# beyzoskaya/HiC-GNN

Measured on AMD Instinct MI355X. Metric: training steps/sec (GATNetSelectiveResidualsUpdated, fwd+loss+bwd+Adam), higher is better.
Workload: dtype fp32; 1 GPU; synth-20000; n_nodes=20000, nnz_with_self_loops=4019956, d=512, heads=2, loss=mse, parallelism=single, gemm=fp32 MFMA

## Files before the change

### hic-gnn_amd/csrc/gat_bwd.hip

```cpp
#include <algorithm>
#include <cstdlib>

#include "gat_agg.hpp"
#include "gat_launch.hpp"

namespace hicgat {

__global__ __launch_bounds__(256) void agg_bwd_dst_h2c256_kernel(
    const int *__restrict__ rowptr, const int *__restrict__ col, int row_begin, int row_end,
    const float *__restrict__ h, const float *__restrict__ a_src, const float *__restrict__ a_dst,
    const float *__restrict__ dout, float ns, float *__restrict__ row_stats) {
  const int i = row_begin + xcd_remap(blockIdx.x, gridDim.x) * 4 + wave_in_block();
  if (i < row_end) agg_bwd_dst_row<2, 256>(i, rowptr, col, h, a_src, a_dst, dout, ns, row_stats);
}

template <int H, int C>
__global__ __launch_bounds__(256) void agg_bwd_dst_generic_kernel(
    const int *__restrict__ rowptr, const int *__restrict__ col, int row_begin, int row_end,
    const float *__restrict__ h, const float *__restrict__ a_src, const float *__restrict__ a_dst,
    const float *__restrict__ dout, float ns, float *__restrict__ row_stats) {
  const int i = row_begin + xcd_remap(blockIdx.x, gridDim.x) * 4 + wave_in_block();
  if (i >= row_end) return;
  agg_bwd_dst_row<H, C>(i, rowptr, col, h, a_src, a_dst, dout, ns, row_stats);
}

template <bool SPLIT = false, bool REMAP = true, class... MK>
__global__ __launch_bounds__(256) void agg_bwd_src_h2c256_kernel(
    const int *__restrict__ rowptr, const int *__restrict__ col, int row_begin, int row_end,
    const float *__restrict__ h, const float *__restrict__ a_src, const float *__restrict__ a_dst,
    const float *__restrict__ row_stats, int64_t ldr, const float *__restrict__ dout, int64_t ldq,
    const float *__restrict__ att_s, const float *__restrict__ att_d, float ns,
    float *__restrict__ dh, float *__restrict__ da_src, MK... mk) {
  const int r = row_begin + (REMAP ? xcd_remap(blockIdx.x, gridDim.x) : (int)blockIdx.x) * 4 + wave_in_block();
  if (r < row_end)
    agg_bwd_src_row<2, 256, SPLIT, sizeof...(MK) != 0>(r, rowptr, col, h, a_src, a_dst, row_stats, ldr, dout, ldq,
                                                       att_s, att_d, ns, dh, da_src, mk...);
}

template <int H, int C, bool REMAP, class... MK>
__global__ __launch_bounds__(256) void agg_bwd_src_generic_kernel(
    const int *__restrict__ rowptr, const int *__restrict__ col, int row_begin, int row_end,
    const float *__restrict__ h, const float *__restrict__ a_src, const float *__restrict__ a_dst,
    const float *__restrict__ row_stats, int64_t ldr, const float *__restrict__ dout, int64_t ldq,
    const float *__restrict__ att_s, const float *__restrict__ att_d, float ns,
    float *__restrict__ dh, float *__restrict__ da_src, MK... mk) {
  const int r = row_begin + (REMAP ? xcd_remap(blockIdx.x, gridDim.x) : (int)blockIdx.x) * 4 + wave_in_block();
  if (r >= row_end) return;
  agg_bwd_src_row<H, C, false, sizeof...(MK) != 0>(r, rowptr, col, h, a_src, a_dst, row_stats, ldr, dout, ldq, att_s,
                                                   att_d, ns, dh, da_src, mk...);
}

template <int ACT>
__global__ __launch_bounds__(256) void agg_bwd_rows_kernel(int row_begin, int row_end,
                                                           const float *__restrict__ g,
                                                           const float *__restrict__ y,
                                                           const float *__restrict__ bias,
                                                           const float *__restrict__ out2,
                                                           float *__restrict__ dout, int64_t ldq,
                                                           float *__restrict__ row_stats) {
  const int i = row_begin + blockIdx.x * 4 + wave_in_block();
  if (i < row_end) agg_bwd_rows_row<2, 256, ACT>(i, g, y, bias, out2, dout, ldq, row_stats);
}

template <int H, int C, int ACT>
__global__ __launch_bounds__(256) void agg_bwd_rows_generic_kernel(int row_begin, int row_end,
                                                                   const float *__restrict__ g,
                                                                   const float *__restrict__ y,
                                                                   const float *__restrict__ bias,
                                                                   const float *__restrict__ out2,
                                                                   float *__restrict__ dout, int64_t ldq,
                                                                   float *__restrict__ row_stats) {
  const int i = row_begin + blockIdx.x * 4 + wave_in_block();
  if (i >= row_end) return;
  agg_bwd_rows_row<H, C, ACT>(i, g, y, bias, out2, dout, ldq, row_stats);
}

constexpr int kParamBlocks = 512;

template <int PARTS>
__global__ __launch_bounds__(256) void param_grad_stage1(const float *__restrict__ h,
                                                         const float *__restrict__ dout,
                                                         const float *__restrict__ da_src,
                                                         const float *__restrict__ row_stats, int N,
                                                         int H, int C, int rows_per_block,
                                                         float *__restrict__ part) {
  constexpr bool kS = PARTS & 1, kT = PARTS & 2, kB = PARTS & 4;
  constexpr int P = (int)kS + (int)kT + (int)kB;
  const int D = H * C, Q = D / 4;
  const int r0 = blockIdx.x * rows_per_block, r1 = min(N, r0 + rows_per_block);
  const float4 *h4 = reinterpret_cast<const float4 *>(h);
  const float4 *g4 = reinterpret_cast<const float4 *>(dout);
  float4 *p4 = reinterpret_cast<float4 *>(part + (size_t)blockIdx.x * P * D);
  for (int q = threadIdx.x; q < Q; q += blockDim.x) {
    const int hd = (4 * q) / C;
    float4 s = make_float4(0.f, 0.f, 0.f, 0.f), t = s, b = s;
#pragma unroll 4
    for (int n = r0; n < r1; ++n) {
      if (kS || kT) {
        const float4 hv = h4[(size_t)n * Q + q];
        if (kS) s = f4_fma(da_src[(size_t)n * H + hd], hv, s);
        if (kT) t = f4_fma(row_stats[(size_t)n * 4 * H + 3 * H + hd], hv, t);
      }
      if (kB) {
        const float4 gv = g4[(size_t)n * Q + q];
        b.x += gv.x; b.y += gv.y; b.z += gv.z; b.w += gv.w;
      }
    }
    int o = 0;
    if (kS) p4[(o++) * Q + q] = s;
    if (kT) p4[(o++) * Q + q] = t;
    if (kB) p4[o * Q + q] = b;
  }
}

constexpr int kPG2Groups = 16, kPG2Cols = 16;
struct PGOut {
  float *o[3];
};
__global__ __launch_bounds__(256) void param_grad_stage2(const float *__restrict__ part, int nblk, int P, int D,
                                                         PGOut out, int accumulate) {
  __shared__ float red[kPG2Groups][kPG2Cols];
  const int cl = threadIdx.x % kPG2Cols, grp = threadIdx.x / kPG2Cols;
  const int c = blockIdx.x * kPG2Cols + cl;
  float s = 0.f;
  if (c < P * D) {
    constexpr int kMax = (kParamBlocks + kPG2Groups - 1) / kPG2Groups;
    float v[kMax];
#pragma unroll
    for (int i = 0; i < kMax; ++i) {
      const int b = grp + i * kPG2Groups;
      v[i] = b < nblk ? part[(size_t)b * P * D + c] : 0.f;
    }
#pragma unroll
    for (int i = 0; i < kMax; ++i) s += v[i];
  }
  red[grp][cl] = s;
  __syncthreads();
  if (grp == 0 && c < P * D) {
    float t = red[0][cl];
#pragma unroll
    for (int g = 1; g < kPG2Groups; ++g) t += red[g][cl];
    float *o = out.o[c / D] + c % D;
    *o = t + (accumulate ? *o : 0.f);
  }
}

constexpr size_t kSrcOccLds = 32768;

int agg_bwd_src_split_launch(const int *rowptr_s, const int *col_s, int row_begin, int row_end, const float *h,
                             const float *a_src, const float *a_dst, const float *row_stats, int64_t ldr,
                             const float *dout, int64_t ldq4, float ns, float *dh, float *da_src, hipStream_t s) {
  hipLaunchKernelGGL((agg_bwd_src_h2c256_kernel<true>), dim3((row_end - row_begin + 3) / 4), dim3(256), 0, s,
                     rowptr_s, col_s, row_begin, row_end, h, a_src, a_dst, row_stats, ldr, dout, ldq4, nullptr, nullptr,
                     ns, dh, da_src);
  HICGAT_CHECK_LAUNCH();
  return HICGAT_OK;
}

template <class... MK>
int agg_bwd_src_launch(const int *rowptr, const int *col, int H, int C, int row_begin, int row_end, const float *h,
                       const float *a_src, const float *a_dst, const float *row_stats, int64_t ldr, const float *dout,
                       int64_t ldq4, const float *att_s, const float *att_d, float ns, float *dh, float *da_src,
                       bool remap, hipStream_t s, MK... mk) {
  const dim3 grid((row_end - row_begin + 3) / 4), block(256);
  return for_gat_shape(H, C, [&](auto shape) {
    return with_flags(
        [&](auto rm) {
          using S = decltype(shape);
          constexpr bool REMAP = rm.value;
          if constexpr (S::h2c256)
            hipLaunchKernelGGL((agg_bwd_src_h2c256_kernel<false, REMAP, MK...>), grid, block,
                               REMAP && !sizeof...(MK) ? kSrcOccLds : 0, s, rowptr, col, row_begin, row_end, h, a_src,
                               a_dst, row_stats, ldr, dout, ldq4, att_s, att_d, ns, dh, da_src, mk...);
          else
            hipLaunchKernelGGL((agg_bwd_src_generic_kernel<S::H, S::C, REMAP, MK...>), grid, block, 0, s, rowptr, col,
                               row_begin, row_end, h, a_src, a_dst, row_stats, ldr, dout, ldq4, att_s, att_d, ns, dh,
                               da_src, mk...);
          HICGAT_CHECK_LAUNCH();
          return HICGAT_OK;
        },
        remap);
  });
}

static int agg_bwd_src_checked(const int32_t *rowptr, const int32_t *col, int N, int H, int C, int row_begin,
                               int row_end, const float *h, const float *a_src, const float *a_dst,
                               const float *row_stats, int64_t ld_stats, const float *dout, int64_t ld_dout,
                               const float *att_src, const float *att_dst, float neg_slope, float *dh, float *da_src,
                               int flags, const AttnMaskArgs *mk, hipStream_t s) {
  if (flags & ~HICGAT_SRC_ROUND_ROBIN) return HICGAT_EINVAL;
  const bool remap = !(flags & HICGAT_SRC_ROUND_ROBIN);
  if (N < 0 || row_begin < 0 || row_end > N || row_begin > row_end) return HICGAT_EINVAL;
  if (!gat_shape_supported(H, C)) return HICGAT_EUNSUPPORTED;
  if (ld_stats < 4 * H || ld_stats % 4 || ld_dout < H * C || ld_dout % 4) return HICGAT_EINVAL;
  if (row_end == row_begin) return HICGAT_OK;
  if (!rowptr || !col || !h || !a_src || !a_dst || !row_stats || !dout || !att_src || !att_dst ||
      !dh || !da_src)
    return HICGAT_EINVAL;
  if (mk)
    return agg_bwd_src_launch(rowptr, col, H, C, row_begin, row_end, h, a_src, a_dst, row_stats, ld_stats, dout,
                              ld_dout / 4, att_src, att_dst, neg_slope, dh, da_src, remap, s, *mk);
  return agg_bwd_src_launch(rowptr, col, H, C, row_begin, row_end, h, a_src, a_dst, row_stats, ld_stats, dout,
                            ld_dout / 4, att_src, att_dst, neg_slope, dh, da_src, remap, s);
}

}

using namespace hicgat;

extern "C" int hicgat_gat_agg_bwd_dst(const int32_t *rowptr, const int32_t *col, int N, int H,
                                      int C, int row_begin, int row_end, const float *h,
                                      const float *a_src, const float *a_dst, const float *dout,
                                      float neg_slope, float *row_stats, hicgat_stream_t stream) {
  if (N < 0 || row_begin < 0 || row_end > N || row_begin > row_end) return HICGAT_EINVAL;
  if (!gat_shape_supported(H, C)) return HICGAT_EUNSUPPORTED;
  if (row_end == row_begin) return HICGAT_OK;
  if (!rowptr || !col || !h || !a_src || !a_dst || !dout || !row_stats) return HICGAT_EINVAL;
  const dim3 grid((row_end - row_begin + 3) / 4), block(256);
  hipStream_t s = (hipStream_t)stream;
  return for_gat_shape(H, C, [&](auto shape) {
    using S = decltype(shape);
    if constexpr (S::h2c256)
      hipLaunchKernelGGL(agg_bwd_dst_h2c256_kernel, grid, block, 0, s, rowptr, col, row_begin, row_end, h, a_src, a_dst,
                         dout, neg_slope, row_stats);
    else
      hipLaunchKernelGGL((agg_bwd_dst_generic_kernel<S::H, S::C>), grid, block, 0, s, rowptr, col, row_begin, row_end,
                         h, a_src, a_dst, dout, neg_slope, row_stats);
    HICGAT_CHECK_LAUNCH();
    return HICGAT_OK;
  });
}

extern "C" int hicgat_gat_agg_bwd_src(const int32_t *rowptr, const int32_t *col, int N, int H,
                                      int C, int row_begin, int row_end, const float *h,
                                      const float *a_src, const float *a_dst,
                                      const float *row_stats, int64_t ld_stats, const float *dout,
                                      int64_t ld_dout, const float *att_src, const float *att_dst,
                                      float neg_slope, float *dh, float *da_src, int flags,
                                      hicgat_stream_t stream) {
  return agg_bwd_src_checked(rowptr, col, N, H, C, row_begin, row_end, h, a_src, a_dst, row_stats, ld_stats, dout,
                             ld_dout, att_src, att_dst, neg_slope, dh, da_src, flags, nullptr, (hipStream_t)stream);
}

extern "C" int hicgat_gat_agg_drop_bwd_src(const int32_t *rowptr, const int32_t *col, int N, int H, int C,
                                           int row_begin, int row_end, const float *h, const float *a_src,
                                           const float *a_dst, const float *row_stats, int64_t ld_stats,
                                           const float *dout, int64_t ld_dout, const float *att_src,
                                           const float *att_dst, float neg_slope, float *dh, float *da_src,
                                           int flags, double p, uint64_t seed, const int64_t *step_counter,
                                           int64_t step_value, uint32_t site, hicgat_stream_t stream) {
  if (!p_ok(p) || !attn_site_ok(site) || misaligned(step_counter, 8)) return HICGAT_EINVAL;
  const AttnMaskArgs mk = attn_mask_args(p, seed, step_counter, step_value, site);
  return agg_bwd_src_checked(rowptr, col, N, H, C, row_begin, row_end, h, a_src, a_dst, row_stats, ld_stats, dout,
                             ld_dout, att_src, att_dst, neg_slope, dh, da_src, flags, &mk, (hipStream_t)stream);
}

extern "C" int hicgat_gat_agg_bwd_rows(int N, int H, int C, int row_begin, int row_end, int act,
                                       const float *g, const float *y, const float *bias,
                                       const float *out2, float *dout, int64_t ld_dout,
                                       float *row_stats, hicgat_stream_t stream) {
  if (N < 0 || row_begin < 0 || row_end > N || row_begin > row_end) return HICGAT_EINVAL;
  if (act && (ld_dout < (int64_t)H * C || ld_dout % 4)) return HICGAT_EINVAL;
  if (act != 0 && act != 1) return HICGAT_EINVAL;
  if (!gat_shape_supported(H, C)) return HICGAT_EUNSUPPORTED;
  if (row_end == row_begin) return HICGAT_OK;
  if (!g || !y || !bias || !out2 || !row_stats || (act && !dout)) return HICGAT_EINVAL;
  const dim3 grid((row_end - row_begin + 3) / 4), block(256);
  hipStream_t s = (hipStream_t)stream;
  const int64_t ldq4 = act ? ld_dout / 4 : 0;
  return for_gat_shape(H, C, [&](auto shape) {
    return with_flags(
        [&](auto relu) {
          using S = decltype(shape);
          constexpr int ACT = relu.value;
          if constexpr (S::h2c256)
            hipLaunchKernelGGL(agg_bwd_rows_kernel<ACT>, grid, block, 0, s, row_begin, row_end, g, y, bias, out2, dout,
                               ldq4, row_stats);
          else
            hipLaunchKernelGGL((agg_bwd_rows_generic_kernel<S::H, S::C, ACT>), grid, block, 0, s, row_begin, row_end, g,
                               y, bias, out2, dout, ldq4, row_stats);
          HICGAT_CHECK_LAUNCH();
          return HICGAT_OK;
        },
        act != 0);
  });
}

extern "C" size_t hicgat_gat_param_grad_workspace_bytes(int N, int D) {
  (void)N;
  return (size_t)kParamBlocks * 3 * (size_t)(D > 0 ? D : 0) * sizeof(float);
}

extern "C" int hicgat_gat_param_grad(const float *h, const float *dout, const float *da_src,
                                     const float *row_stats, int N, int H, int C, float *datt_src,
                                     float *datt_dst, float *dbias, int accumulate, void *workspace,
                                     size_t workspace_bytes, hicgat_stream_t stream) {
  if (N < 0 || H <= 0 || C <= 0 || (C % 4) != 0) return HICGAT_EINVAL;
  const int D = H * C;
  const int parts = (datt_src ? 1 : 0) | (datt_dst ? 2 : 0) | (dbias ? 4 : 0);
  if (!parts || !workspace) return HICGAT_EINVAL;
  if (((parts & 3) && !h) || ((parts & 1) && !da_src) || ((parts & 2) && !row_stats) || ((parts & 4) && !dout))
    return HICGAT_EINVAL;
  if (workspace_bytes < hicgat_gat_param_grad_workspace_bytes(N, D)) return HICGAT_EINVAL;
  const int rpb = N > 0 ? (N + kParamBlocks - 1) / kParamBlocks : 1;
  const int nblk = N > 0 ? (N + rpb - 1) / rpb : 0;
  float *part = static_cast<float *>(workspace);
  PGOut out{};
  int P = 0;
  if (datt_src) out.o[P++] = datt_src;
  if (datt_dst) out.o[P++] = datt_dst;
  if (dbias) out.o[P++] = dbias;
  hipStream_t s = (hipStream_t)stream;
  if (nblk > 0) {
    static constexpr decltype(&param_grad_stage1<1>) kStage1[8] = {
        nullptr,
        param_grad_stage1<1>, param_grad_stage1<2>, param_grad_stage1<3>, param_grad_stage1<4>,
        param_grad_stage1<5>, param_grad_stage1<6>, param_grad_stage1<7>};
    hipLaunchKernelGGL(kStage1[parts], dim3(nblk), dim3(128), 0, s, h, dout, da_src, row_stats, N, H, C, rpb, part);
    HICGAT_CHECK_LAUNCH();
  }
  hipLaunchKernelGGL(param_grad_stage2, dim3((P * D + kPG2Cols - 1) / kPG2Cols), dim3(kPG2Cols * kPG2Groups), 0, s,
                     part, nblk, P, D, out, accumulate);
  HICGAT_CHECK_LAUNCH();
  return HICGAT_OK;
}
```

Measured before the change: 587.6 steps/s.

## Software-pipeline param-grad reduction with batched loads, split groups, wave-uniform weights

Rewrites stage 1 of the attention/bias parameter-gradient reduction. Rows are now processed in double-buffered batches of loads so memory latency overlaps the FMAs. The h-weighted sums and the dout bias sum run in separate 128-thread groups. When C is a multiple of 256, per-head weights are loaded once per wave and broadcast with readlane. Stage 2 now issues its loads unconditionally with clamped indices and prefetches the old output value. This adds register pressure and extra code paths, and it only touches a small reduction inside the full training step.

New measurement: 589.7 steps/s (median of 6 runs). No clear change (+0.3%).

```diff
diff --git a/hic-gnn_amd/csrc/gat_bwd.hip b/hic-gnn_amd/csrc/gat_bwd.hip
--- a/hic-gnn_amd/csrc/gat_bwd.hip
+++ b/hic-gnn_amd/csrc/gat_bwd.hip
@@ -77,7 +77,88 @@
 
 constexpr int kParamBlocks = 512;
 
-template <int PARTS>
+constexpr int kPGLanes = 128;
+#ifndef HICGAT_PG_BATCH
+#define HICGAT_PG_BATCH 8
+#endif
+constexpr int kPGBatch = HICGAT_PG_BATCH;
+
+template <bool UNI>
+struct PGWeights {
+  float w[UNI ? 1 : kPGBatch];
+  __device__ __forceinline__ void load(const float *__restrict__ x, int ld, int hd, int n, int last) {
+    if constexpr (UNI) {
+      w[0] = x[(size_t)min(n + (int)(threadIdx.x % 64 % kPGBatch), last) * ld + hd];
+    } else {
+#pragma unroll
+      for (int i = 0; i < kPGBatch; ++i) w[i] = x[(size_t)min(n + i, last) * ld + hd];
+    }
+  }
+  __device__ __forceinline__ float get(int i) const {
+    if constexpr (UNI)
+      return __int_as_float(__builtin_amdgcn_readlane(__float_as_int(w[0]), i));
+    else
+      return w[i];
+  }
+};
+
+template <bool kS, bool kT, bool UNI>
+struct PGBatch {
+  float4 v[kPGBatch];
+  PGWeights<UNI> a, d;
+  __device__ __forceinline__ void load(const float4 *__restrict__ x4, const float *__restrict__ wsrc,
+                                       const float *__restrict__ wdst, int H, int Q, int q, int hd, int n,
+                                       int last) {
+#pragma unroll
+    for (int i = 0; i < kPGBatch; ++i) v[i] = x4[(size_t)min(n + i, last) * Q + q];
+    if (kS) a.load(wsrc, H, hd, n, last);
+    if (kT) d.load(wdst, 4 * H, hd, n, last);
+  }
+  __device__ __forceinline__ void add(int i, float4 &s, float4 &t) const {
+    if (kS) s = f4_fma(a.get(i), v[i], s);
+    if (kT) t = f4_fma(d.get(i), v[i], t);
+    if (!kS && !kT) {
+      s.x += v[i].x; s.y += v[i].y; s.z += v[i].z; s.w += v[i].w;
+    }
+  }
+};
+
+template <bool kS, bool kT, bool UNI>
+__device__ __forceinline__ void pg_group_cols(const float4 *__restrict__ x4, const float *__restrict__ wsrc,
+                                              const float *__restrict__ wdst, int H, int C, int Q, int r0, int r1,
+                                              int lane, float4 *__restrict__ p4) {
+  constexpr int K = kPGBatch;
+  const int last = r1 - 1;
+  for (int q = lane; q < Q; q += kPGLanes) {
+    const int hd = UNI ? __builtin_amdgcn_readfirstlane((4 * q) / C) : (4 * q) / C;
+    float4 s = make_float4(0.f, 0.f, 0.f, 0.f), t = s;
+    PGBatch<kS, kT, UNI> A, B;
+    int n = r0;
+    A.load(x4, wsrc, wdst, H, Q, q, hd, n, last);
+    for (; n + 2 * K <= r1; n += 2 * K) {
+      B.load(x4, wsrc, wdst, H, Q, q, hd, n + K, last);
+#pragma unroll
+      for (int i = 0; i < K; ++i) A.add(i, s, t);
+      A.load(x4, wsrc, wdst, H, Q, q, hd, n + 2 * K, last);
+#pragma unroll
+      for (int i = 0; i < K; ++i) B.add(i, s, t);
+    }
+    const int rem = r1 - n;
+    if (rem > K) B.load(x4, wsrc, wdst, H, Q, q, hd, n + K, last);
+#pragma unroll
+    for (int i = 0; i < K; ++i)
+      if (i < rem) A.add(i, s, t);
+    if (rem > K) {
+#pragma unroll
+      for (int i = 0; i < K; ++i)
+        if (K + i < rem) B.add(i, s, t);
+    }
+    if (kS || !kT) p4[q] = s;
+    if (kT) p4[(kS ? Q : 0) + q] = t;
+  }
+}
+
+template <int PARTS, bool UNI>
 __global__ __launch_bounds__(256) void param_grad_stage1(const float *__restrict__ h,
                                                          const float *__restrict__ dout,
                                                          const float *__restrict__ da_src,
@@ -85,31 +166,21 @@
                                                          int H, int C, int rows_per_block,
                                                          float *__restrict__ part) {
   constexpr bool kS = PARTS & 1, kT = PARTS & 2, kB = PARTS & 4;
-  constexpr int P = (int)kS + (int)kT + (int)kB;
+  constexpr int PA = (int)kS + (int)kT, P = PA + (int)kB;
   const int D = H * C, Q = D / 4;
   const int r0 = blockIdx.x * rows_per_block, r1 = min(N, r0 + rows_per_block);
-  const float4 *h4 = reinterpret_cast<const float4 *>(h);
-  const float4 *g4 = reinterpret_cast<const float4 *>(dout);
+  if (r0 >= r1) return;
   float4 *p4 = reinterpret_cast<float4 *>(part + (size_t)blockIdx.x * P * D);
-  for (int q = threadIdx.x; q < Q; q += blockDim.x) {
-    const int hd = (4 * q) / C;
-    float4 s = make_float4(0.f, 0.f, 0.f, 0.f), t = s, b = s;
-#pragma unroll 4
-    for (int n = r0; n < r1; ++n) {
-      if (kS || kT) {
-        const float4 hv = h4[(size_t)n * Q + q];
-        if (kS) s = f4_fma(da_src[(size_t)n * H + hd], hv, s);
-        if (kT) t = f4_fma(row_stats[(size_t)n * 4 * H + 3 * H + hd], hv, t);
-      }
-      if (kB) {
-        const float4 gv = g4[(size_t)n * Q + q];
-        b.x += gv.x; b.y += gv.y; b.z += gv.z; b.w += gv.w;
-      }
-    }
-    int o = 0;
-    if (kS) p4[(o++) * Q + q] = s;
-    if (kT) p4[(o++) * Q + q] = t;
-    if (kB) p4[o * Q + q] = b;
+  const int group = threadIdx.x / kPGLanes, lane = threadIdx.x % kPGLanes;
+  if constexpr (PA != 0) {
+    if (group == 0)
+      pg_group_cols<kS, kT, UNI>(reinterpret_cast<const float4 *>(h), da_src, kT ? row_stats + 3 * H : nullptr, H, C,
+                                 Q, r0, r1, lane, p4);
+  }
+  if constexpr (kB) {
+    if (group == (PA != 0 ? 1 : 0))
+      pg_group_cols<false, false, false>(reinterpret_cast<const float4 *>(dout), nullptr, nullptr, H, C, Q, r0, r1,
+                                         lane, p4 + PA * Q);
   }
 }
 
@@ -123,16 +194,18 @@
   const int cl = threadIdx.x % kPG2Cols, grp = threadIdx.x / kPG2Cols;
   const int c = blockIdx.x * kPG2Cols + cl;
   float s = 0.f;
+  float *o = out.o[min(c, P * D - 1) / D] + min(c, P * D - 1) % D;
+  const float old = *o;
   if (c < P * D) {
     constexpr int kMax = (kParamBlocks + kPG2Groups - 1) / kPG2Groups;
     float v[kMax];
 #pragma unroll
     for (int i = 0; i < kMax; ++i) {
       const int b = grp + i * kPG2Groups;
-      v[i] = b < nblk ? part[(size_t)b * P * D + c] : 0.f;
+      v[i] = part[(size_t)max(min(b, nblk - 1), 0) * P * D + c];
     }
 #pragma unroll
-    for (int i = 0; i < kMax; ++i) s += v[i];
+    for (int i = 0; i < kMax; ++i) s += grp + i * kPG2Groups < nblk ? v[i] : 0.f;
   }
   red[grp][cl] = s;
   __syncthreads();
@@ -140,8 +213,7 @@
     float t = red[0][cl];
 #pragma unroll
     for (int g = 1; g < kPG2Groups; ++g) t += red[g][cl];
-    float *o = out.o[c / D] + c % D;
-    *o = t + (accumulate ? *o : 0.f);
+    *o = t + (accumulate ? old : 0.f);
   }
 }
 
@@ -312,11 +384,18 @@
   if (dbias) out.o[P++] = dbias;
   hipStream_t s = (hipStream_t)stream;
   if (nblk > 0) {
-    static constexpr decltype(&param_grad_stage1<1>) kStage1[8] = {
-        nullptr,
-        param_grad_stage1<1>, param_grad_stage1<2>, param_grad_stage1<3>, param_grad_stage1<4>,
-        param_grad_stage1<5>, param_grad_stage1<6>, param_grad_stage1<7>};
-    hipLaunchKernelGGL(kStage1[parts], dim3(nblk), dim3(128), 0, s, h, dout, da_src, row_stats, N, H, C, rpb, part);
+    using Stage1 = decltype(&param_grad_stage1<1, false>);
+    static constexpr Stage1 kStage1[2][8] = {
+        {nullptr, param_grad_stage1<1, false>, param_grad_stage1<2, false>, param_grad_stage1<3, false>,
+         param_grad_stage1<4, false>, param_grad_stage1<5, false>, param_grad_stage1<6, false>,
+         param_grad_stage1<7, false>},
+        {nullptr, param_grad_stage1<1, true>, param_grad_stage1<2, true>, param_grad_stage1<3, true>,
+         param_grad_stage1<4, true>, param_grad_stage1<5, true>, param_grad_stage1<6, true>,
+         param_grad_stage1<7, true>}};
+    const bool uni = C % 256 == 0;
+    const int groups = ((parts & 3) ? 1 : 0) + ((parts & 4) ? 1 : 0);
+    hipLaunchKernelGGL(kStage1[uni][parts], dim3(nblk), dim3(kPGLanes * groups), 0, s, h, dout, da_src, row_stats, N,
+                       H, C, rpb, part);
     HICGAT_CHECK_LAUNCH();
   }
   hipLaunchKernelGGL(param_grad_stage2, dim3((P * D + kPG2Cols - 1) / kPG2Cols), dim3(kPG2Cols * kPG2Groups), 0, s,
```
